# XinMing0411/AC-VAE

Measured on AMD Instinct MI355X. Metric: train-step captions/s (and audio-sec/s) at B=32, 1/2/4/8 MI355X, higher is better.
Workload: dtype f32

## Files before the change

### acvae_amd/csrc/conv.h

```cpp
#pragma once
#include <hip/hip_runtime.h>
#include <stdint.h>
#include "common.h"
#include "job_table.h"
#include "bn_bwd.h"

struct DropoutSpec {
  float p;
  const uint8_t* mask;
  uint64_t seed;
  uint32_t site;
};

enum { UP_PLAIN = 0, UP_POOL = 1, UP_DROP = 2 };

namespace acvae {
int conv3x3_igemm(const float* X, const float* scale, const float* shift, const float* Wp, float* Y, float* partials,
                  int N, int H, int W, int Cin, int Cout, hipStream_t st);
int conv_partials_rows(int N, int H, int W);
int conv3x3_igemm_bf16(const bf16_t* X, const float* scale, const float* shift, const bf16_t* Wp, bf16_t* Y,
                       float* partials, int N, int H, int W, int Cin, int Cout, hipStream_t st);
long conv3x3_wgrad_bf16_slab_floats(int N, int H, int W, int Cin, int Cout);
int conv3x3_wgrad_bf16_splits(int N, int H, int W, int Cin, int Cout);
int conv3x3_wgrad_bf16_launch(const bf16_t* dY, const bf16_t* X, const float* scale, const float* shift, float* slab, int N,
                              int H, int W, int Cin, int Cout, hipStream_t st);
int wgrad_reduce(const float* slab, int nsplit, float* dW_oihw, int Cout, int Cin, hipStream_t st);
long conv3x3_wgrad_slab_floats(int N, int H, int W, int Cin, int Cout);
int conv3x3_wgrad(const float* dY, const float* X, const float* scale, const float* shift, float* dW_oihw, float* slab,
                  int N, int H, int W, int Cin, int Cout, hipStream_t st);
bool conv3x3_wino_ok(int H, int W, int Cin, int Cout);
long conv3x3_wino_weight_floats(int Cin, int Cout);
int conv_wino_partials_rows(int N, int H, int W);
int conv3x3_wino_weights(const float* W_oihw, float* U, int Cout, int Cin, bool dgrad, hipStream_t st);
struct WinoWeightsJob { const float* W; float* U; int Cout, Cin, dgrad; };
using WinoWeightsBatch = RangeTable<WinoWeightsJob, 32>;
int conv3x3_wino_weights_batch(WinoWeightsBatch& b, hipStream_t st);
struct WinoBnReduce { const float* Y; const float* scale; const float* shift; const float* mean; const float* invstd; };
int conv3x3_wino(const float* X, const float* scale, const float* shift, const float* U, float* Y, float* partials, int N,
                 int H, int W, int Cin, int Cout, hipStream_t st, const WinoBnReduce* red = nullptr);
bool conv3x3_wino_wgrad_ok(int H, int W, int Cin, int Cout);
long conv3x3_wino_wgrad_slab_floats(int N, int H, int W, int Cin, int Cout);
int conv3x3_wino_wgrad(const float* dY, const float* X, const float* scale, const float* shift, float* dW_oihw, float* slab,
                       int N, int H, int W, int Cin, int Cout, hipStream_t st);
template <class T>
int repack_weights(const float* W_oihw, T* Wf, T* Wd, int Cout, int Cin, hipStream_t st);
struct RepackJob { const float* W; void* dst; int Cout, Cin, dgrad; };
using RepackBatch = RangeTable<RepackJob, 32>;
template <class T>
int repack_weights_batch(RepackBatch& b, hipStream_t st);
inline int conv3x3_igemm(const bf16_t* X, const float* scale, const float* shift, const bf16_t* Wp, bf16_t* Y,
                         float* partials, int N, int H, int W, int Cin, int Cout, hipStream_t st) {
  return conv3x3_igemm_bf16(X, scale, shift, Wp, Y, partials, N, H, W, Cin, Cout, st);
}
inline int conv3x3_wgrad(const bf16_t* dY, const bf16_t* X, const float* scale, const float* shift, float* dW_oihw,
                         float* slab, int N, int H, int W, int Cin, int Cout, hipStream_t st) {
  int r = conv3x3_wgrad_bf16_launch(dY, X, scale, shift, slab, N, H, W, Cin, Cout, st);
  if (r != 0) return r;
  return wgrad_reduce(slab, conv3x3_wgrad_bf16_splits(N, H, W, Cin, Cout), dW_oihw, Cout, Cin, st);
}
template <class T>
inline long conv3x3_wgrad_slab_floats_t(int N, int H, int W, int Cin, int Cout) {
  return sizeof(T) == 2 ? conv3x3_wgrad_bf16_slab_floats(N, H, W, Cin, Cout) : conv3x3_wgrad_slab_floats(N, H, W, Cin, Cout);
}
int bn0_stats(const float* x, float* partials, long rows, int F, int* nparts, hipStream_t st);
int bn0_partials_rows(long rows);
int bn_finalize(const float* partials, int P, int C, double count, const float* gamma, const float* beta,
                float* running_mean, float* running_var, int64_t* nbt, int training, float* scale, float* shift,
                float* mean, float* invstd, double* dpart, hipStream_t st);
long colsum_scratch_doubles(int width);
int colsum_tickets_reset(double* dpart, hipStream_t st);
long colsum_ticket_words();
int colsum2(const float* x, int P, int width, double* dpart, float* out, float* out2, int split, hipStream_t st);
struct ColsumJob { const float* x; int P, width; float* out; float* out_b; int R; long d0; };
using ColsumBatch = RangeTable<ColsumJob, 6, int>;
int colsum_batch(ColsumBatch& b, double* dpart, long dpart_doubles, hipStream_t st);
bool colsum_batch_plan(ColsumBatch& b, long dpart_doubles, long* dsum_doubles);
int conv1_first_blocks(int N, int T);
template <class TY>
int conv1_first_fwd(const float* x, const float* scale0, const float* shift0, const float* W1, TY* Y,
                    float* partials, int N, int T, int F, hipStream_t st);
template <class TY>
int conv1_first_bwd(const float* x, const float* scale0, const float* shift0, const float* mean0, const float* invstd0,
                    const float* W1, const TY* dY, float* dw_part, float* bn_part, float* dW1, float* dgamma0,
                    float* dbeta0, double* dpart, int N, int T, int F, hipStream_t st, const BnBwdApply* bn = nullptr);
template <class T>
int bn_relu_pool(const T* Y, const float* scale, const float* shift, T* P, int N, int H, int W, int C,
                 DropoutSpec drop, hipStream_t st, bool pool = true);
int bn_bwd_blocks(int N, int H, int W, int C);
template <class T>
int bn_bwd(const T* Y, const T* dO, int upstream, const float* scale, const float* shift, const float* mean,
           const float* invstd, float* partials, float* sum_g, float* sum_gy, T* dY, double* dpart, int N, int H,
           int W, int C, DropoutSpec drop, hipStream_t st, bool batch_stats = true, int ready_rows = 0);
template <class T>
int bn_bwd_sums(const T* Y, const T* dO, int upstream, const float* scale, const float* shift, const float* mean,
                const float* invstd, float* partials, float* sum_g, float* sum_gy, double* dpart, int N, int H, int W, int C,
                DropoutSpec drop, hipStream_t st, int ready_rows = 0);
template <class T>
int relu_mask(const T* Y, const float* scale, const float* shift, uint8_t* out, int N, int H, int W, int C, hipStream_t st);
template <class T>
int freq_mean(const T* P, float* out, long rows, int Fp, int C, hipStream_t st);
template <class T>
int freq_mean_bwd(const float* dae, T* dP, long rows, int Fp, int C, hipStream_t st);
int time_pool(const float* ae, float* out, int N, int S, int C, DropoutSpec drop, hipStream_t st);
int relu_dropout(float* x, int total, DropoutSpec drop, hipStream_t st);
}

int acvae_gemm_nt_dual(const float* A1, int64_t lda1, const float* B1, int64_t ldb1, int K1, const float* A2,
                       int64_t lda2, const float* B2, int64_t ldb2, int K2, const float* bias, float* C, int64_t ldc,
                       int M, int N, int accumulate, hipStream_t st, float* skws = nullptr);
int acvae_gemm_nt_pair(const float* A0, int64_t lda0, const float* B0, int64_t ldb0, int K0, const float* bias0, float* C0,
                       int64_t ldc0, int N0, int acc0, const float* A1, int64_t lda1, const float* B1, int64_t ldb1, int K1,
                       const float* bias1, float* C1, int64_t ldc1, int N1, int acc1, int M, hipStream_t st);
constexpr int TN_TICKETS = 256;
int acvae_gemm_tn_fused(const float* A, int64_t lda, const float* B, int64_t ldb, float* C, int64_t ldc, int M, int N, int K,
                        int accumulate, float* ws, int64_t ws_bytes, hipStream_t st);
struct TnJob {
  const float* A; long lda; const float* B; long ldb; float* C; long ldc;
  int M, N, K, k_per, slices, gx, gy, tk0;
  long slab0;
};
using TnGroup = acvae::RangeTable<TnJob, 8, int>;
bool acvae_gemm_tn_group_add(TnGroup& g, const float* A, long lda, const float* B, long ldb, float* C, long ldc, int M, int N,
                             int K);
long acvae_gemm_tn_group_plan(TnGroup& g);
int acvae_gemm_tn_group(TnGroup& g, float* ws, int64_t ws_bytes, hipStream_t st);
long acvae_skinny_ws_floats();
// ... 6 lines not shown
```

### acvae_amd/csrc/conv.hip

```cpp
#include "mfma_tile.h"
#include "../../include/acvae_hip.h"
#include "conv.h"
#include "prof.h"

namespace {
using namespace mfma;

struct FastDiv {
  unsigned long long mul;
  static FastDiv make(int d) { return FastDiv{((1ULL << 40) + (unsigned long long)d - 1) / (unsigned long long)d}; }
  __device__ __forceinline__ int div(int x) const { return (int)(((unsigned long long)(unsigned)x * mul) >> 40); }
};

struct ConvKMajorLoader {
  const float* X;
  const float* scale;
  const float* shift;
  int H, W, C, M, NC;
  FastDiv dW, dH;
  int dy, dx, ci;
  bool colok;
  float4 sc, sh;
  template <int WT>
  __device__ __forceinline__ void init(int col0) {
// ... 474 lines not shown
template <class T>
__global__ void repack_dgrad_kernel(const float* __restrict__ W, T* __restrict__ Wd, int Cout, int Cin) {
  const long total = (long)Cout * Cin * 9;
  for (long i = blockIdx.x * (long)blockDim.x + threadIdx.x; i < total; i += (long)gridDim.x * blockDim.x) {
    const int ci = (int)(i / (9 * Cout)), rem = (int)(i % (9 * Cout));
    const int tp = rem / Cout, co = rem % Cout;
    Wd[i] = (T)W[((long)co * Cin + ci) * 9 + (8 - tp)];
  }
}

template <class T>
__global__ void repack_batch_kernel(acvae::RepackBatch b) {
  const long total = b.start[b.n];
  for (long i = blockIdx.x * (long)blockDim.x + threadIdx.x; i < total; i += (long)gridDim.x * blockDim.x) {
    const int l = b.find(i);
    const acvae::RepackJob& job = b.job[l];
    const long k = i - b.start[l];
    const int Cout = job.Cout, Cin = job.Cin;
    const float* W = job.W;
    T* out = reinterpret_cast<T*>(job.dst);
    if (!job.dgrad) {
      const int co = (int)(k / (9 * Cin)), rem = (int)(k % (9 * Cin));
      const int tap = rem / Cin, ci = rem % Cin;
      out[k] = (T)W[((long)co * Cin + ci) * 9 + tap];
    } else {
      const int ci = (int)(k / (9 * Cout)), rem = (int)(k % (9 * Cout));
      const int tp = rem / Cout, co = rem % Cout;
      out[k] = (T)W[((long)co * Cin + ci) * 9 + (8 - tp)];
    }
  }
}

__global__ __launch_bounds__(256) void bn0_stats_kernel(const float* __restrict__ x, float* __restrict__ partials,
                                                        long rows, int F, int rows_per_block) {
  __shared__ float red[2][4][64];
  const int w = threadIdx.x & 63, g = threadIdx.x >> 6;
  const long r0 = (long)blockIdx.x * rows_per_block;
  float s = 0.f, q = 0.f;
  if (w < F)
    for (long r = r0 + g; r < r0 + rows_per_block && r < rows; r += 4) {
      const float v = x[r * F + w];
      s += v; q += v * v;
    }
  red[0][g][w] = s; red[1][g][w] = q;
  __syncthreads();
  if (threadIdx.x < 64 && w < F) {
    float* out = partials + (long)blockIdx.x * 2 * F;
    out[w] = red[0][0][w] + red[0][1][w] + red[0][2][w] + red[0][3][w];
    out[F + w] = red[1][0][w] + red[1][1][w] + red[1][2][w] + red[1][3][w];
  }
}

constexpr int CS_R = 64;
constexpr int CS_TICKETS = 128;
inline int cs_groups(int P) { return P < 1 ? 1 : P < 16 ? P : P <= 1024 ? 16 : P <= 4096 ? 32 : CS_R; }

struct BnFinalizeArgs {
  double count;
  const float *gamma, *beta;
  float *running_mean, *running_var;
  int64_t* nbt;
  float *scale, *shift, *mean_out, *invstd_out;
};

__device__ __forceinline__ void cs_store(double* p, double v) {
  __hip_atomic_store(reinterpret_cast<unsigned long long*>(p), (unsigned long long)__double_as_longlong(v), __ATOMIC_RELAXED,
                     __HIP_MEMORY_SCOPE_AGENT);
}
__device__ __forceinline__ double cs_load(const double* p) {
  return __longlong_as_double((long long)__hip_atomic_load(reinterpret_cast<const unsigned long long*>(p), __ATOMIC_RELAXED,
                                                           __HIP_MEMORY_SCOPE_AGENT));
}
__device__ __forceinline__ bool cs_last_arriver(unsigned* ticket, unsigned expect, int* s_last) {
  asm volatile("s_waitcnt vmcnt(0)" ::: "memory");
  __syncthreads();
  if (threadIdx.x == 0) {
    const unsigned prev = __hip_atomic_fetch_add(ticket, 1u, __ATOMIC_RELAXED, __HIP_MEMORY_SCOPE_AGENT);
    const int last = prev == expect - 1u;
    if (last) __hip_atomic_store(ticket, 0u, __ATOMIC_RELAXED, __HIP_MEMORY_SCOPE_AGENT);
    *s_last = last;
  }
  __syncthreads();
  return *s_last != 0;
}

template <bool FINALIZE>
__global__ __launch_bounds__(256) void colsum_kernel(const float* __restrict__ partials, int P, int width, double* __restrict__ dpart,
                                                     float* __restrict__ out, float* __restrict__ out2, int split,
                                                     BnFinalizeArgs bn) {
  __shared__ double red[4][64];
  __shared__ int s_last;
  unsigned* tickets = reinterpret_cast<unsigned*>(dpart);
  double* dsum = dpart + CS_TICKETS / 2;
  const int il = threadIdx.x & 63, g = threadIdx.x >> 6;
  const int i = blockIdx.x * 64 + il;
  const int R = gridDim.y;
  double a = 0.0;
  if (i < width)
    for (int p = blockIdx.y + g * R; p < P; p += 4 * R) a += (double)partials[(long)p * width + i];
  red[g][il] = a;
  __syncthreads();
  if (g == 0 && i < width) cs_store(dsum + (long)blockIdx.y * width + i, red[0][il] + red[1][il] + red[2][il] + red[3][il]);
  if (!FINALIZE) {
    if (!cs_last_arriver(tickets + blockIdx.x, (unsigned)R, &s_last)) return;
    if (g != 0 || i >= width) return;
    double t = 0.0;
    for (int r0 = 0; r0 < R; r0 += 8) {
      double v[8];
#pragma unroll
      for (int u = 0; u < 8; ++u) v[u] = r0 + u < R ? cs_load(dsum + (long)(r0 + u) * width + i) : 0.0;
#pragma unroll
      for (int u = 0; u < 8; ++u)
        if (r0 + u < R) t += v[u];
    }
    if (split > 0 && i >= split) out2[i - split] = (float)t;
    else out[i] = (float)t;
  } else {
    const int C = width >> 1, cb = C >> 6;
    const int xc = blockIdx.x % cb;
    if (!cs_last_arriver(tickets + xc, (unsigned)(2 * R), &s_last)) return;
    if (g != 0) return;
    const int c = xc * 64 + il;
    double sm = 0.0, q = 0.0;
    for (int r0 = 0; r0 < R; r0 += 8) {
      double v[8], w[8];
#pragma unroll
      for (int u = 0; u < 8; ++u) {
        v[u] = r0 + u < R ? cs_load(dsum + (long)(r0 + u) * width + c) : 0.0;
        w[u] = r0 + u < R ? cs_load(dsum + (long)(r0 + u) * width + C + c) : 0.0;
      }
#pragma unroll
      for (int u = 0; u < 8; ++u)
        if (r0 + u < R) { sm += v[u]; q += w[u]; }
    }
    const double mean = sm / bn.count;
    double var = q / bn.count - mean * mean;
    if (var < 0.0) var = 0.0;
    const float invstd = (float)(1.0 / sqrt(var + 1e-5));
    const float sc = bn.gamma[c] * invstd;
    bn.scale[c] = sc; bn.shift[c] = bn.beta[c] - (float)mean * sc;
    bn.mean_out[c] = (float)mean; bn.invstd_out[c] = invstd;
    const double unbiased = bn.count > 1.0 ? var * bn.count / (bn.count - 1.0) : var;
    bn.running_mean[c] = 0.9f * bn.running_mean[c] + 0.1f * (float)mean;
    bn.running_var[c] = 0.9f * bn.running_var[c] + 0.1f * (float)unbiased;
    if (c == 0 && bn.nbt) bn.nbt[0] += 1;
  }
}

__global__ __launch_bounds__(256) void colsum_batch_kernel(acvae::ColsumBatch b, double* __restrict__ dpart) {
  __shared__ double red[4][64];
  __shared__ int s_last;
  const int j = b.find((int)blockIdx.x);
  const acvae::ColsumJob& job = b.job[j];
  const int R = job.R;
  if ((int)blockIdx.y >= R) return;
  const float* __restrict__ partials = job.x;
  const int P = job.P, width = job.width;
  unsigned* tickets = reinterpret_cast<unsigned*>(dpart);
  double* dsum = dpart + CS_TICKETS / 2 + job.d0;
  const int il = threadIdx.x & 63, g = threadIdx.x >> 6;
  const int i = ((int)blockIdx.x - b.start[j]) * 64 + il;
  double a = 0.0;
  if (i < width)
    for (int p = blockIdx.y + g * R; p < P; p += 4 * R) a += (double)partials[(long)p * width + i];
  red[g][il] = a;
  __syncthreads();
  if (g == 0 && i < width) cs_store(dsum + (long)blockIdx.y * width + i, red[0][il] + red[1][il] + red[2][il] + red[3][il]);
  if (!cs_last_arriver(tickets + blockIdx.x, (unsigned)R, &s_last)) return;
  if (g != 0 || i >= width) return;
  double t = 0.0;
  for (int r0 = 0; r0 < R; r0 += 8) {
    double v[8];
#pragma unroll
    for (int u = 0; u < 8; ++u) v[u] = r0 + u < R ? cs_load(dsum + (long)(r0 + u) * width + i) : 0.0;
#pragma unroll
    for (int u = 0; u < 8; ++u)
      if (r0 + u < R) t += v[u];
  }
  job.out[i] = (float)t;
  if (job.out_b) job.out_b[i] = (float)t;
}

__global__ __launch_bounds__(64) void bn_eval_kernel(int C, const float* __restrict__ gamma, const float* __restrict__ beta,
                                                     const float* __restrict__ running_mean, const float* __restrict__ running_var,
                                                     float* __restrict__ scale, float* __restrict__ shift,
                                                     float* __restrict__ mean_out, float* __restrict__ invstd_out) {
  const int c = blockIdx.x * 64 + threadIdx.x;
  if (c >= C) return;
  const float invstd = 1.0f / sqrtf(running_var[c] + 1e-5f);
  const float sc = gamma[c] * invstd;
  scale[c] = sc; shift[c] = beta[c] - running_mean[c] * sc;
  mean_out[c] = running_mean[c]; invstd_out[c] = invstd;
}

constexpr int C1_RB = 8;
template <class TY>
__global__ __launch_bounds__(256) void conv1_first_fwd_kernel(const float* __restrict__ x,
                                                              const float* __restrict__ scale0,
                                                              const float* __restrict__ shift0,
                                                              const float* __restrict__ W1, TY* __restrict__ Y,
                                                              float* __restrict__ partials, int T, int F) {
  __shared__ float wl[64 * 9];
  __shared__ float patch[(C1_RB + 2) * 66];
  __shared__ float red[2][16][64];
  const int nblk_t = (T + C1_RB - 1) / C1_RB;
  const int n = blockIdx.x / nblk_t, t0 = (blockIdx.x % nblk_t) * C1_RB;
  for (int i = threadIdx.x; i < 64 * 9; i += 256) wl[i] = W1[i];
  for (int i = threadIdx.x; i < (C1_RB + 2) * 66; i += 256) {
    const int r = i / 66, cidx = i % 66;
    const int t = t0 + r - 1, w = cidx - 1;
    float v = 0.f;
    if (t >= 0 && t < T && w >= 0 && w < F) v = x[((long)n * T + t) * F + w] * scale0[w] + shift0[w];
    patch[i] = v;
  }
  __syncthreads();
  const int cq = threadIdx.x & 15, pp = threadIdx.x >> 4;
  float wreg[4][9];
#pragma unroll
  for (int c = 0; c < 4; ++c)
#pragma unroll
    for (int k = 0; k < 9; ++k) wreg[c][k] = wl[(cq * 4 + c) * 9 + k];
  float s[4] = {0, 0, 0, 0}, q[4] = {0, 0, 0, 0};
  for (int pix = pp; pix < C1_RB * 64; pix += 16) {
    const int r = pix >> 6, w = pix & 63;
    const int t = t0 + r;
    if (t >= T || w >= F) continue;
    float in[9];
#pragma unroll
    for (int k = 0; k < 9; ++k) in[k] = patch[(r + k / 3) * 66 + w + k % 3];
    float o[4];
#pragma unroll
// ... 606 lines not shown
  }
  prof_end(ACVAE_PROF_CONV_WGRAD, st);
  hipLaunchKernelGGL(wgrad_reduce_kernel, dim3(ew_grid((long)Cout * NC)), dim3(256), 0, st, slab,
                     s * wgrad_slabs_per_slice(NC, Cout), dW_oihw, Cout, Cin);
  ACVAE_LAUNCH_CHECK();
  return ACVAE_OK;
}

int wgrad_reduce(const float* slab, int nsplit, float* dW_oihw, int Cout, int Cin, hipStream_t st) {
  hipLaunchKernelGGL(wgrad_reduce_kernel, dim3(ew_grid((long)Cout * 9 * Cin)), dim3(256), 0, st, slab, nsplit, dW_oihw, Cout,
                     Cin);
  ACVAE_LAUNCH_CHECK();
  return ACVAE_OK;
}

template <class T>
int repack_weights(const float* W_oihw, T* Wf, T* Wd, int Cout, int Cin, hipStream_t st) {
  const long total = (long)Cout * Cin * 9;
  if (Wf) hipLaunchKernelGGL(repack_fwd_kernel<T>, dim3(ew_grid(total)), dim3(256), 0, st, W_oihw, Wf, Cout, Cin);
  if (Wd) hipLaunchKernelGGL(repack_dgrad_kernel<T>, dim3(ew_grid(total)), dim3(256), 0, st, W_oihw, Wd, Cout, Cin);
  ACVAE_LAUNCH_CHECK();
  return ACVAE_OK;
}
template int repack_weights<float>(const float*, float*, float*, int, int, hipStream_t);
template int repack_weights<bf16_t>(const float*, bf16_t*, bf16_t*, int, int, hipStream_t);
template <class T>
int repack_weights_batch(RepackBatch& b, hipStream_t st) {
  if (!b.ok()) return ACVAE_EINVAL;
  if (b.n <= 0) return ACVAE_OK;
  for (int l = 0; l < b.n; ++l)
    if (!b.job[l].W || !b.job[l].dst) return ACVAE_EINVAL;
  const long total = b.seal([](const RepackJob& j) { return (long)j.Cout * j.Cin * 9; });
  hipLaunchKernelGGL(repack_batch_kernel<T>, dim3(cdiv(total, 256) > 8192 ? 8192 : cdiv(total, 256)), dim3(256), 0, st, b);
  ACVAE_LAUNCH_CHECK();
  return ACVAE_OK;
}
template int repack_weights_batch<float>(RepackBatch&, hipStream_t);
template int repack_weights_batch<bf16_t>(RepackBatch&, hipStream_t);

int bn0_stats(const float* x, float* partials, long rows, int F, int* nparts, hipStream_t st) {
  if (F > 64) return ACVAE_EUNSUPPORTED;
  const int rpb = 256;
  const int nb = cdiv(rows, rpb);
  hipLaunchKernelGGL(bn0_stats_kernel, dim3(nb), dim3(256), 0, st, x, partials, rows, F, rpb);
  *nparts = nb;
  ACVAE_LAUNCH_CHECK();
  return ACVAE_OK;
}
int bn0_partials_rows(long rows) { return cdiv(rows, 256); }

int colsum2(const float* partials, int P, int width, double* dpart, float* out, float* out2, int split,
            hipStream_t st) {
  if (cdiv(width, 64) > CS_TICKETS) return ACVAE_EUNSUPPORTED;
  const int R = cs_groups(P);
  hipLaunchKernelGGL(colsum_kernel<false>, dim3(cdiv(width, 64), R), dim3(256), 0, st, partials, P, width, dpart, out, out2, split,
                     BnFinalizeArgs{});
  ACVAE_LAUNCH_CHECK();
  return ACVAE_OK;
}
bool colsum_batch_plan(ColsumBatch& b, long dpart_doubles, long* dsum_doubles) {
  long d = 0;
  for (int j = 0; j < b.n; ++j) {
    ColsumJob& c = b.job[j];
    c.R = cs_groups(c.P);
    c.d0 = d;
    d += (long)c.R * c.width;
  }
  const int blocks = b.seal([](const ColsumJob& c) { return cdiv(c.width, 64); });
  if (dsum_doubles) *dsum_doubles = d;
  return !(b.n == 1 || blocks > CS_TICKETS || CS_TICKETS / 2 + d > dpart_doubles);
}
int colsum_batch(ColsumBatch& b, double* dpart, long dpart_doubles, hipStream_t st) {
  if (!b.ok()) return ACVAE_EINVAL;
  if (b.n <= 0) return ACVAE_OK;
  if (!colsum_batch_plan(b, dpart_doubles, nullptr)) {
    for (int j = 0; j < b.n; ++j) {
      const ColsumJob& c = b.job[j];
      ACVAE_TRY(colsum2(c.x, c.P, c.width, dpart, c.out, nullptr, 0, st));
      if (c.out_b) ACVAE_TRY(colsum2(c.x, c.P, c.width, dpart, c.out_b, nullptr, 0, st));
    }
    return ACVAE_OK;
  }
  int maxr = 1;
  for (int j = 0; j < b.n; ++j)
    if (b.job[j].R > maxr) maxr = b.job[j].R;
  hipLaunchKernelGGL(colsum_batch_kernel, dim3(b.start[b.n], maxr), dim3(256), 0, st, b, dpart);
  ACVAE_LAUNCH_CHECK();
  return ACVAE_OK;
}
long colsum_scratch_doubles(int width) { return CS_TICKETS / 2 + (long)CS_R * width; }
long colsum_ticket_words() { return CS_TICKETS; }
int colsum_tickets_reset(double* dpart, hipStream_t st) {
  return hipMemsetAsync(dpart, 0, CS_TICKETS * sizeof(unsigned), st) == hipSuccess ? ACVAE_OK : (int)hipGetLastError();
}

int bn_finalize(const float* partials, int P, int C, double count, const float* gamma, const float* beta,
                float* running_mean, float* running_var, int64_t* nbt, int training, float* scale, float* shift,
                float* mean, float* invstd, double* dpart, hipStream_t st) {
  if (training) {
    if (C % 64 != 0 || cdiv(2 * C, 64) > CS_TICKETS) return ACVAE_EUNSUPPORTED;
    const int R = cs_groups(P);
    hipLaunchKernelGGL(colsum_kernel<true>, dim3(2 * C / 64, R), dim3(256), 0, st, partials, P, 2 * C, dpart, nullptr, nullptr, 0,
                       BnFinalizeArgs{count, gamma, beta, running_mean, running_var, nbt, scale, shift, mean, invstd});
  } else {
    hipLaunchKernelGGL(bn_eval_kernel, dim3(cdiv(C, 64)), dim3(64), 0, st, C, gamma, beta, running_mean, running_var, scale,
                       shift, mean, invstd);
  }
  ACVAE_LAUNCH_CHECK();
  return ACVAE_OK;
}

int conv1_first_blocks(int N, int T) { return N * cdiv(T, C1_RB); }
template <class TY>
int conv1_first_fwd(const float* x, const float* scale0, const float* shift0, const float* W1, TY* Y,
                    float* partials, int N, int T, int F, hipStream_t st) {
  if (F != 64) return ACVAE_EUNSUPPORTED;
  hipLaunchKernelGGL(conv1_first_fwd_kernel<TY>, dim3(conv1_first_blocks(N, T)), dim3(256), 0, st, x, scale0, shift0, W1,
                     Y, partials, T, F);
  ACVAE_LAUNCH_CHECK();
  return ACVAE_OK;
}
template int conv1_first_fwd<float>(const float*, const float*, const float*, const float*, float*, float*, int, int, int, hipStream_t);
template int conv1_first_fwd<bf16_t>(const float*, const float*, const float*, const float*, bf16_t*, float*, int, int, int, hipStream_t);
template <class TY>
int conv1_first_bwd(const float* x, const float* scale0, const float* shift0, const float* mean0, const float* invstd0,
                    const float* W1, const TY* dY, float* dw_part, float* bn_part, float* dW1, float* dgamma0,
                    float* dbeta0, double* dpart, int N, int T, int F, hipStream_t st, const BnBwdApply* bn) {
  if (F != 64) return ACVAE_EUNSUPPORTED;
  const int nb = conv1_first_blocks(N, T);
  if (bn) {
    if (!std::is_same<TY, float>::value) return ACVAE_EUNSUPPORTED;
    hipLaunchKernelGGL((conv1_first_bwd_kernel<float, true>), dim3(nb), dim3(256), 0, st, x, scale0, shift0, mean0, invstd0, W1,
                       (const float*)dY, dw_part, bn_part, T, F, *bn);
  } else {
    hipLaunchKernelGGL((conv1_first_bwd_kernel<TY, false>), dim3(nb), dim3(256), 0, st, x, scale0, shift0, mean0, invstd0, W1, dY,
                       dw_part, bn_part, T, F, BnBwdApply{});
  }
  ACVAE_LAUNCH_CHECK();
  ACVAE_TRY(colsum2(dw_part, nb, 576, dpart, dW1, nullptr, 0, st));
  ACVAE_TRY(colsum2(bn_part, nb, 128, dpart, dbeta0, dgamma0, 64, st));
  return ACVAE_OK;
}
template int conv1_first_bwd<float>(const float*, const float*, const float*, const float*, const float*, const float*, const float*, float*, float*, float*, float*, float*, double*, int, int, int, hipStream_t, const BnBwdApply*);
template int conv1_first_bwd<bf16_t>(const float*, const float*, const float*, const float*, const float*, const float*, const bf16_t*, float*, float*, float*, float*, float*, double*, int, int, int, hipStream_t, const BnBwdApply*);

template <class T>
int bn_relu_pool(const T* Y, const float* scale, const float* shift, T* P, int N, int H, int W, int C,
                 DropoutSpec drop, hipStream_t st, bool pool) {
  const long total = pool ? (long)N * (H / 2) * (W / 2) * (C / 4) : (long)N * H * W * (C / 4);
  if (total <= 0 || C % 4 != 0) return ACVAE_EINVAL;
  if (pool)
    hipLaunchKernelGGL(bn_relu_pool_kernel<T>, dim3(ew_grid(total)), dim3(256), 0, st, Y, scale, shift, P, N, H, W, C, drop);
  else
    hipLaunchKernelGGL(bn_relu_drop_kernel<T>, dim3(ew_grid(total)), dim3(256), 0, st, Y, scale, shift, P, N, H, W, C, drop);
  ACVAE_LAUNCH_CHECK();
// ... 124 lines not shown
```

### acvae_amd/csrc/ops_abi.hip

```cpp
#include "common.h"
#include "conv.h"
#include "rnn.h"
#include "../../include/acvae_hip.h"

namespace {
inline long al64(long x) { return (x + 63) & ~63L; }

struct ConvWs {
  long wp, partials, dpart, slab, total;
};
ConvWs conv_ws(int N, int H, int W, int Cin, int Cout) {
  ConvWs w;
  long o = 0;
  w.wp = o; o = al64(o + (long)Cout * 16 * Cin);
  long part = Cin == 1 ? (long)acvae::conv1_first_blocks(N, H) * 128 : (long)acvae::conv_partials_rows(N, H, W) * 2 * Cout;
  if (Cin > 1 && W >= 4 && W % 2 == 0 && (long)acvae::conv_wino_partials_rows(N, H, W) * 2 * Cout > part)
    part = (long)acvae::conv_wino_partials_rows(N, H, W) * 2 * Cout;
  w.partials = o; o = al64(o + part);
  w.dpart = o; o = al64(o + 2 * acvae::colsum_scratch_doubles(2 * Cout > 1024 ? 2 * Cout : 1024));
  long slab = Cin == 1 ? (long)acvae::conv1_first_blocks(N, H) * (576 + 128)
                       : acvae::conv3x3_wgrad_slab_floats(N, H, W, Cin, Cout);
  if (Cin % 64 == 0) {
    const long sb = acvae::conv3x3_wgrad_bf16_slab_floats(N, H, W, Cin, Cout);
    if (sb > slab) slab = sb;
// ... 358 lines not shown

extern "C" int acvae_lstm_step(const float* x, const float* h, const float* c, const float* w_ih, const float* w_hh,
                               const float* b_ih, const float* b_hh, float* h_out, float* c_out, void* ws_v,
                               int64_t ws_bytes, int N, int I, int H, void* stream) {
  if (N <= 0 || I <= 0 || H <= 0 || !x || !h || !c || !w_ih || !w_hh || !h_out || !c_out || !ws_v) return ACVAE_EINVAL;
  if (ws_bytes < acvae_rnn_workspace_bytes(N, 1, I, H)) return ACVAE_EWORKSPACE;
  hipStream_t st = (hipStream_t)stream;
  float* ws = (float*)ws_v;
  float* sk = ws;
  float* gates = ws + al64(acvae_skinny_ws_floats());
  ACVAE_TRY(acvae_skinny_ws_reset(sk, st));
  ACVAE_TRY(acvae_gemm_nt_dual(x, I, w_ih, I, I, nullptr, 0, nullptr, 0, 0, b_ih, gates, 4 * H, N, 4 * H, 0, st, sk));
  ACVAE_TRY(acvae_gemm_nt_dual(h, H, w_hh, H, H, nullptr, 0, nullptr, 0, 0, b_hh, gates, 4 * H, N, 4 * H, 1, st, sk));
  return acvae::lstm_fwd(gates, 4 * H, c, H, h_out, H, c_out, H, nullptr, 0, N, H, st);
}

extern "C" int acvae_bigru_seq(const float* X, const int64_t* lens, const void* const* w, float* hidden, void* ws_v,
                               int64_t ws_bytes, int N, int Tc, int E, int H, void* stream) {
  if (N <= 0 || Tc <= 0 || E <= 0 || H <= 0 || !X || !lens || !w || !hidden || !ws_v) return ACVAE_EINVAL;
  for (int i = 0; i < 8; ++i)
    if (!w[i]) return ACVAE_EINVAL;
  if (ws_bytes < acvae_rnn_workspace_bytes(N, Tc, E, H)) return ACVAE_EWORKSPACE;
  hipStream_t st = (hipStream_t)stream;
  const long R = (long)N * Tc;
  float* ws = (float*)ws_v;
  float* sk = ws;
  float* gi = ws + al64(acvae_skinny_ws_floats());
  float* gh = gi + al64(R * 8 * H);
  float* hcur = gh + al64((long)N * 4 * H);
  float* save = hcur + al64((long)N * H);
  float* hps = save + al64(R * 5 * H);
  ACVAE_TRY(acvae_skinny_ws_reset(sk, st));
  for (int dir = 0; dir < 2; ++dir) {
    const float* wih = (const float*)w[dir * 4 + 0];
    const float* whh = (const float*)w[dir * 4 + 1];
    const float* bih = (const float*)w[dir * 4 + 2];
    const float* bhh = (const float*)w[dir * 4 + 3];
    ACVAE_TRY(acvae_gemm_nt_dual(X, E, wih, E, E, nullptr, 0, nullptr, 0, 0, bih, gi, 3 * H, (int)R, 3 * H, 0, st, sk));
    ACVAE_TRY(acvae::copy_rows(hcur, H, nullptr, 0, N, H, st));
    for (int k = 0; k < Tc; ++k) {
      const int t = dir ? Tc - 1 - k : k;
      ACVAE_TRY(acvae_gemm_nt_dual(hcur, H, whh, H, H, nullptr, 0, nullptr, 0, 0, bhh, gh, 3 * H, N, 3 * H, 0, st, sk));
      ACVAE_TRY(acvae::gru_fwd(gi + (long)t * 3 * H, (long)Tc * 3 * H, gh, 3 * H, hcur, H, hcur, H,
                               hidden + (long)t * 2 * H + dir * H, (long)Tc * 2 * H, save + (long)t * 4 * H,
                               (long)Tc * 4 * H, hps + (long)t * H, (long)Tc * H, lens, t, N, H, st));
    }
  }
  return ACVAE_OK;
}

extern "C" int64_t acvae_colsum_workspace_bytes(int cols) {
  return cols > 0 ? al64(2 * acvae::colsum_scratch_doubles(cols)) * 4 : -1;
}
extern "C" int acvae_colsum(const float* x, int rows, int cols, float* out, void* ws, int64_t ws_bytes, void* stream) {
  if (!x || !out || !ws || rows <= 0 || cols <= 0) return ACVAE_EINVAL;
  if (ws_bytes < acvae_colsum_workspace_bytes(cols)) return ACVAE_EWORKSPACE;
  ACVAE_TRY(acvae::colsum_tickets_reset((double*)ws, (hipStream_t)stream));
  return acvae::colsum2(x, rows, cols, (double*)ws, out, nullptr, 0, (hipStream_t)stream);
}

static int colsum_table(int n, const int* P, const int* width, acvae::ColsumBatch& b) {
  if (n <= 0 || n > acvae::ColsumBatch::capacity || !P || !width) return ACVAE_EINVAL;
  for (int j = 0; j < n; ++j) {
    if (P[j] <= 0 || width[j] <= 0) return ACVAE_EINVAL;
    b.add({nullptr, P[j], width[j], nullptr, nullptr, 0, 0});
  }
  return ACVAE_OK;
}
extern "C" int64_t acvae_colsum_batch_workspace_bytes(int n, const int* P, const int* width) {
  acvae::ColsumBatch b;
  if (colsum_table(n, P, width, b) != ACVAE_OK) return -1;
  long d = 0;
  acvae::colsum_batch_plan(b, 0, &d);
  return ((int64_t)acvae::colsum_ticket_words() / 2 + d) * 8;
}
extern "C" int acvae_colsum_batch_plan(int n, const int* P, const int* width, int64_t ws_bytes) {
  acvae::ColsumBatch b;
  ACVAE_TRY(colsum_table(n, P, width, b));
  return acvae::colsum_batch_plan(b, (long)(ws_bytes / 8), nullptr) ? 1 : 0;
}
extern "C" int acvae_colsum_batch(int n, const void* const* x, const int* P, const int* width, const void* const* out,
                                  const void* const* out_b, void* ws, int64_t ws_bytes, int reset_tickets, void* stream) {
  acvae::ColsumBatch b;
  ACVAE_TRY(colsum_table(n, P, width, b));
  if (!x || !out || !ws) return ACVAE_EINVAL;
  for (int j = 0; j < n; ++j) {
    if (!x[j] || !out[j]) return ACVAE_EINVAL;
    b.job[j].x = (const float*)x[j];
    b.job[j].out = (float*)out[j];
    b.job[j].out_b = out_b ? (float*)out_b[j] : nullptr;
  }
  acvae::ColsumBatch plan = b;
  acvae::colsum_batch_plan(plan, 0, nullptr);
  for (int j = 0; j < n; ++j)
    if (ws_bytes < ((int64_t)acvae::colsum_ticket_words() / 2 + (int64_t)plan.job[j].R * width[j]) * 8) return ACVAE_EWORKSPACE;
  hipStream_t st = (hipStream_t)stream;
  if (reset_tickets) ACVAE_TRY(acvae::colsum_tickets_reset((double*)ws, st));
  return acvae::colsum_batch(b, (double*)ws, (long)(ws_bytes / 8), st);
}
```

### include/acvae_hip.h

```cpp
#ifndef ACVAE_HIP_H
#define ACVAE_HIP_H
#include <stdint.h>
#ifdef __cplusplus
extern "C" {
#endif

#define ACVAE_ABI_VERSION 3
int acvae_abi_version(void);

#define ACVAE_FLAG_NO_PERSIST 1
#define ACVAE_FLAG_DEFER_PARAM_GRADS 2
#define ACVAE_FLAG_NO_ATTN_SPLIT 4
#define ACVAE_FLAG_ROLLOUT_GRAD 16
#define ACVAE_FLAG_TEST_STALL 8

int acvae_persist_status_register(int device, void* status_words_host);

int acvae_gemm_nt(const float* A, int64_t lda, const float* B, int64_t ldb, const float* bias, float* C,
                  int64_t ldc, int M, int N, int K, int accumulate, void* stream);
int acvae_gemm_tn(const float* A, int64_t lda, const float* B, int64_t ldb, float* C, int64_t ldc, int M, int N,
                  int K, int accumulate, float* slab_ws, int64_t slab_ws_bytes, void* stream);
int64_t acvae_gemm_tn_workspace_bytes(int M, int N, int K);
int64_t acvae_colsum_workspace_bytes(int cols);
int acvae_colsum(const float* x, int rows, int cols, float* out, void* ws, int64_t ws_bytes, void* stream);

int64_t acvae_gemm_nt_splitk_workspace_bytes(void);
int acvae_gemm_nt_split_plan(int M, int N, int K1, int K2, int with_ws);
int acvae_gemm_nt_dual_ws(const float* A1, int64_t lda1, const float* B1, int64_t ldb1, int K1, const float* A2,
                          int64_t lda2, const float* B2, int64_t ldb2, int K2, const float* bias, float* C, int64_t ldc,
                          int M, int N, int accumulate, float* ws, int64_t ws_bytes, int reset_tickets, void* stream);
int acvae_gemm_nt_pair_c(const float* A0, int64_t lda0, const float* B0, int64_t ldb0, int K0, const float* bias0, float* C0,
                         int64_t ldc0, int N0, int acc0, const float* A1, int64_t lda1, const float* B1, int64_t ldb1, int K1,
                         const float* bias1, float* C1, int64_t ldc1, int N1, int acc1, int M, void* stream);
int64_t acvae_gemm_tn_fused_workspace_bytes(int M, int N, int K);
int acvae_gemm_tn_fused_plan(int M, int N, int K, int64_t ws_bytes);
int acvae_gemm_tn_fused_c(const float* A, int64_t lda, const float* B, int64_t ldb, float* C, int64_t ldc, int M, int N,
                          int K, int accumulate, float* ws, int64_t ws_bytes, int reset_tickets, void* stream);
int64_t acvae_gemm_tn_group_workspace_bytes(int n, const int* M, const int* N, const int* K);
int acvae_gemm_tn_group_c(int n, const void* const* A, const int64_t* lda, const void* const* B, const int64_t* ldb,
                          const void* const* C, const int64_t* ldc, const int* M, const int* N, const int* K, void* ws,
                          int64_t ws_bytes, int reset_tickets, void* stream);
int64_t acvae_colsum_batch_workspace_bytes(int n, const int* P, const int* width);
int acvae_colsum_batch_plan(int n, const int* P, const int* width, int64_t ws_bytes);
int acvae_colsum_batch(int n, const void* const* x, const int* P, const int* width, const void* const* out,
                       const void* const* out_b, void* ws, int64_t ws_bytes, int reset_tickets, void* stream);
int acvae_transpose(const float* in, int64_t ld_in, float* out, int64_t ld_out, int rows, int cols, void* stream);

int64_t acvae_attn_fwd_workspace_bytes(int N, int Tq, int S, int A, int E);
int acvae_attn_fwd(const float* qproj, int64_t q_sn, int64_t q_sj, const float* encproj, const float* enc,
                   const int64_t* lens, const float* v, float* ctx, int64_t c_sn, int64_t c_sj, float* weights,
                   int64_t w_sn, int64_t w_sj, int N, int Tq, int S, int A, int E, void* ws, int64_t ws_bytes, void* stream,
                   int flags);
int acvae_tanh_att(const float* x, float* y, int64_t n, void* stream);
int64_t acvae_attn_bwd_workspace_bytes(int N, int Tq, int S, int A);
int acvae_attn_bwd(const float* dctx, int64_t dc_sn, int64_t dc_sj, const float* qproj, int64_t q_sn, int64_t q_sj,
                   const float* encproj, const float* enc, const int64_t* lens, const float* v,
                   const float* weights, int64_t w_sn, int64_t w_sj, float* dqproj, int64_t dq_sn, int64_t dq_sj,
                   float* dencproj, float* denc, float* dv_part, float* ws, int64_t ws_bytes, int N, int Tq, int S,
                   int A, int E, void* stream);

int acvae_reparam_fwd(const float* ml, int64_t ld_ml, const float* eps, int64_t ld_eps, float* mean, float* logv,
                      float* z, int64_t ld_out, float* z2, int64_t ld_z2, int rows, int E, void* stream);
int acvae_reparam_bwd(const float* dz, int64_t ld_dz, const float* dmean_ext, const float* dlog_ext, int64_t ld_ext,
                      const float* logv, int64_t ld_lv, const float* eps, int64_t ld_eps, float* dml, int64_t ld_dml,
                      int rows, int E, void* stream);

int64_t acvae_kl_partials(int64_t n_elem);
int acvae_gauss_kl_fwd(const float* mu1, const float* lv1, const float* mu2, const float* lv2, float* partials,
                       float* out_scalar, int64_t rows, int E, void* stream);
int acvae_gauss_kl_bwd(const float* mu1, const float* lv1, const float* mu2, const float* lv2, const float* grad_out,
                       float* dmu1, float* dlv1, float* dmu2, float* dlv2, int64_t rows, int E, void* stream);

int acvae_row_logsoftmax_argmax(const float* logits, int64_t ld_n, int64_t ld_t, int64_t* argmax, float* max_logprob,
                                float* lse, int64_t o_sn, int64_t o_st, int N, int T, int V, void* stream);
#define ACVAE_SAMPLE_GREEDY 0
#define ACVAE_SAMPLE_GUMBEL 1
// ... 318 lines not shown
```

Measured before the change: 2131.

## Rework column-sum reduction with float4 row slots, contiguous row ranges and split finalize

Reworks the column-sum/BN-finalize kernels. Each group now owns a contiguous row range and reads it with float4 loads across 16-64 row slots, with an 8-deep batch of loads issued ahead. A grid z-dimension splits columns when a group has many rows, and the last-arriver finalize now reduces the partial sums across all four waves instead of one. The aim is more memory-level parallelism and a faster tail in this reduction, at the cost of larger shared-memory use, more complex ticket counts and a changed summation order.

```diff
diff --git a/acvae_amd/csrc/conv.h b/acvae_amd/csrc/conv.h
--- a/acvae_amd/csrc/conv.h
+++ b/acvae_amd/csrc/conv.h
@@ -67,11 +67,13 @@
 int bn_finalize(const float* partials, int P, int C, double count, const float* gamma, const float* beta,
                 float* running_mean, float* running_var, int64_t* nbt, int training, float* scale, float* shift,
                 float* mean, float* invstd, double* dpart, hipStream_t st);
+struct ColsumPlan { int groups, slots; long scratch; };
+ColsumPlan colsum_plan(int P, int width);
 long colsum_scratch_doubles(int width);
 int colsum_tickets_reset(double* dpart, hipStream_t st);
 long colsum_ticket_words();
 int colsum2(const float* x, int P, int width, double* dpart, float* out, float* out2, int split, hipStream_t st);
-struct ColsumJob { const float* x; int P, width; float* out; float* out_b; int R; long d0; };
+struct ColsumJob { const float* x; int P, width; float* out; float* out_b; int R, sh; long d0; };
 using ColsumBatch = RangeTable<ColsumJob, 6, int>;
 int colsum_batch(ColsumBatch& b, double* dpart, long dpart_doubles, hipStream_t st);
 bool colsum_batch_plan(ColsumBatch& b, long dpart_doubles, long* dsum_doubles);
diff --git a/acvae_amd/csrc/conv.hip b/acvae_amd/csrc/conv.hip
--- a/acvae_amd/csrc/conv.hip
+++ b/acvae_amd/csrc/conv.hip
@@ -550,8 +550,13 @@
 }
 
 constexpr int CS_R = 64;
+constexpr int CS_DEPTH = 8;
 constexpr int CS_TICKETS = 128;
 inline int cs_groups(int P) { return P < 1 ? 1 : P < 16 ? P : P <= 1024 ? 16 : P <= 4096 ? 32 : CS_R; }
+inline int cs_slot_shift(int P) {
+  const int rows = cdiv(P < 1 ? 1 : P, cs_groups(P));
+  return rows <= 16 * CS_DEPTH ? 0 : rows <= 32 * CS_DEPTH ? 1 : 2;
+}
 
 struct BnFinalizeArgs {
   double count;
@@ -582,55 +587,112 @@
   return *s_last != 0;
 }
 
+template <bool VEC>
+__device__ __forceinline__ void cs_slot_sums(const float* __restrict__ x, int r0, int r1, int width, int c0, int s, int slots,
+                                             double (&a)[4]) {
+  const int k1 = c0 + 1 < width ? 1 : 0, k2 = c0 + 2 < width ? 2 : 0, k3 = c0 + 3 < width ? 3 : 0;
+  for (int p = r0 + s; p < r1; p += slots * CS_DEPTH) {
+    float4 v[CS_DEPTH];
+#pragma unroll
+    for (int u = 0; u < CS_DEPTH; ++u) {
+      const int pu = p + u * slots;
+      const float* row = x + (long)(pu < r1 ? pu : p) * width + c0;
+      if (VEC) v[u] = *reinterpret_cast<const float4*>(row);
+      else v[u] = make_float4(row[0], row[k1], row[k2], row[k3]);
+    }
+    __builtin_amdgcn_sched_barrier(0);
+#pragma unroll
+    for (int u = 0; u < CS_DEPTH; ++u) {
+      const bool in = p + u * slots < r1;
+      a[0] += in ? (double)v[u].x : 0.0; a[1] += in ? (double)v[u].y : 0.0;
+      a[2] += in ? (double)v[u].z : 0.0; a[3] += in ? (double)v[u].w : 0.0;
+    }
+  }
+}
+__device__ __forceinline__ void cs_stage1(const float* __restrict__ x, int P, int width, int xb, int sub, int sh, int grp, int R,
+                                          double* __restrict__ dsum, double* red) {
+  const int slots = 16 << sh, cols = 64 >> sh;
+  const int q = threadIdx.x & ((cols >> 2) - 1), s = threadIdx.x >> (4 - sh);
+  const int cbase = xb * 64 + sub * cols;
+  const int c0 = cbase + q * 4;
+  const int per = P / R, rem = P % R;
+  const int r0 = grp * per + (grp < rem ? grp : rem), r1 = r0 + per + (grp < rem ? 1 : 0);
+  double a[4] = {0.0, 0.0, 0.0, 0.0};
+  if (c0 < width) {
+    if ((width & 3) == 0 && (reinterpret_cast<uintptr_t>(x) & 15) == 0) cs_slot_sums<true>(x, r0, r1, width, c0, s, slots, a);
+    else cs_slot_sums<false>(x, r0, r1, width, c0, s, slots, a);
+  }
+#pragma unroll
+  for (int c = 0; c < 4; ++c) red[s * cols + q * 4 + c] = a[c];
+  __syncthreads();
+  const int i = cbase + (int)threadIdx.x;
+  if ((int)threadIdx.x < cols && i < width) {
+    double t = red[threadIdx.x];
+#pragma unroll 8
+    for (int k = 1; k < slots; ++k) t += red[k * cols + threadIdx.x];
+    cs_store(dsum + (long)grp * width + i, t);
+  }
+}
+template <int N>
+__device__ __forceinline__ void cs_quarter(const double* __restrict__ dsum, int R, int width, const int (&col)[N], double (&t)[N]) {
+  const int per = (R + 3) >> 2, w = threadIdx.x >> 6;
+  const int lo = w * per, hi = lo + per < R ? lo + per : R;
+#pragma unroll
+  for (int k = 0; k < N; ++k) t[k] = 0.0;
+  for (int r0 = lo; r0 < hi; r0 += 8) {
+    double v[N][8];
+#pragma unroll
+    for (int u = 0; u < 8; ++u)
+#pragma unroll
+      for (int k = 0; k < N; ++k) v[k][u] = r0 + u < hi ? cs_load(dsum + (long)(r0 + u) * width + col[k]) : 0.0;
+#pragma unroll
+    for (int u = 0; u < 8; ++u)
+      if (r0 + u < hi) {
+#pragma unroll
+        for (int k = 0; k < N; ++k) t[k] += v[k][u];
+      }
+  }
+}
+__device__ __forceinline__ double cs_quarter(const double* __restrict__ dsum, int R, int width, int col) {
+  const int c[1] = {col};
+  double t[1];
+  cs_quarter<1>(dsum, R, width, c, t);
+  return t[0];
+}
+
 template <bool FINALIZE>
 __global__ __launch_bounds__(256) void colsum_kernel(const float* __restrict__ partials, int P, int width, double* __restrict__ dpart,
                                                      float* __restrict__ out, float* __restrict__ out2, int split,
                                                      BnFinalizeArgs bn) {
-  __shared__ double red[4][64];
+  __shared__ double red[16][64];
   __shared__ int s_last;
   unsigned* tickets = reinterpret_cast<unsigned*>(dpart);
   double* dsum = dpart + CS_TICKETS / 2;
   const int il = threadIdx.x & 63, g = threadIdx.x >> 6;
   const int i = blockIdx.x * 64 + il;
-  const int R = gridDim.y;
-  double a = 0.0;
-  if (i < width)
-    for (int p = blockIdx.y + g * R; p < P; p += 4 * R) a += (double)partials[(long)p * width + i];
-  red[g][il] = a;
-  __syncthreads();
-  if (g == 0 && i < width) cs_store(dsum + (long)blockIdx.y * width + i, red[0][il] + red[1][il] + red[2][il] + red[3][il]);
+  const int R = gridDim.y, sh = gridDim.z >> 1;
+  cs_stage1(partials, P, width, blockIdx.x, blockIdx.z, sh, blockIdx.y, R, dsum, &red[0][0]);
   if (!FINALIZE) {
-    if (!cs_last_arriver(tickets + blockIdx.x, (unsigned)R, &s_last)) return;
+    if (!cs_last_arriver(tickets + blockIdx.x, (unsigned)(R << sh), &s_last)) return;
+    red[g][il] = i < width ? cs_quarter(dsum, R, width, i) : 0.0;
+    __syncthreads();
     if (g != 0 || i >= width) return;
-    double t = 0.0;
-    for (int r0 = 0; r0 < R; r0 += 8) {
-      double v[8];
-#pragma unroll
-      for (int u = 0; u < 8; ++u) v[u] = r0 + u < R ? cs_load(dsum + (long)(r0 + u) * width + i) : 0.0;
-#pragma unroll
-      for (int u = 0; u < 8; ++u)
-        if (r0 + u < R) t += v[u];
-    }
+    const double t = red[0][il] + red[1][il] + red[2][il] + red[3][il];
     if (split > 0 && i >= split) out2[i - split] = (float)t;
     else out[i] = (float)t;
   } else {
     const int C = width >> 1, cb = C >> 6;
     const int xc = blockIdx.x % cb;
-    if (!cs_last_arriver(tickets + xc, (unsigned)(2 * R), &s_last)) return;
+    if (!cs_last_arriver(tickets + xc, (unsigned)(2 * R << sh), &s_last)) return;
+    const int c = xc * 64 + il;
+    const int cols[2] = {c, C + c};
+    double t2[2];
+    cs_quarter<2>(dsum, R, width, cols, t2);
+    red[g][il] = t2[0]; red[4 + g][il] = t2[1];
+    __syncthreads();
     if (g != 0) return;
-    const int c = xc * 64 + il;
-    double sm = 0.0, q = 0.0;
-    for (int r0 = 0; r0 < R; r0 += 8) {
-      double v[8], w[8];
-#pragma unroll
-      for (int u = 0; u < 8; ++u) {
-        v[u] = r0 + u < R ? cs_load(dsum + (long)(r0 + u) * width + c) : 0.0;
-        w[u] = r0 + u < R ? cs_load(dsum + (long)(r0 + u) * width + C + c) : 0.0;
-      }
-#pragma unroll
-      for (int u = 0; u < 8; ++u)
-        if (r0 + u < R) { sm += v[u]; q += w[u]; }
-    }
+    const double sm = red[0][il] + red[1][il] + red[2][il] + red[3][il];
+    const double q = red[4][il] + red[5][il] + red[6][il] + red[7][il];
     const double mean = sm / bn.count;
     double var = q / bn.count - mean * mean;
     if (var < 0.0) var = 0.0;
@@ -646,35 +708,24 @@
 }
 
 __global__ __launch_bounds__(256) void colsum_batch_kernel(acvae::ColsumBatch b, double* __restrict__ dpart) {
-  __shared__ double red[4][64];
+  __shared__ double red[16][64];
   __shared__ int s_last;
   const int j = b.find((int)blockIdx.x);
   const acvae::ColsumJob& job = b.job[j];
-  const int R = job.R;
-  if ((int)blockIdx.y >= R) return;
-  const float* __restrict__ partials = job.x;
-  const int P = job.P, width = job.width;
+  const int R = job.R, sh = job.sh;
+  if ((int)blockIdx.y >= R || (int)blockIdx.z >= 1 << sh) return;
+  const int width = job.width;
   unsigned* tickets = reinterpret_cast<unsigned*>(dpart);
   double* dsum = dpart + CS_TICKETS / 2 + job.d0;
   const int il = threadIdx.x & 63, g = threadIdx.x >> 6;
-  const int i = ((int)blockIdx.x - b.start[j]) * 64 + il;
-  double a = 0.0;
-  if (i < width)
-    for (int p = blockIdx.y + g * R; p < P; p += 4 * R) a += (double)partials[(long)p * width + i];
-  red[g][il] = a;
+  const int xb = (int)blockIdx.x - b.start[j];
+  const int i = xb * 64 + il;
+  cs_stage1(job.x, job.P, width, xb, blockIdx.z, sh, blockIdx.y, R, dsum, &red[0][0]);
+  if (!cs_last_arriver(tickets + blockIdx.x, (unsigned)(R << sh), &s_last)) return;
+  red[g][il] = i < width ? cs_quarter(dsum, R, width, i) : 0.0;
   __syncthreads();
-  if (g == 0 && i < width) cs_store(dsum + (long)blockIdx.y * width + i, red[0][il] + red[1][il] + red[2][il] + red[3][il]);
-  if (!cs_last_arriver(tickets + blockIdx.x, (unsigned)R, &s_last)) return;
   if (g != 0 || i >= width) return;
-  double t = 0.0;
-  for (int r0 = 0; r0 < R; r0 += 8) {
-    double v[8];
-#pragma unroll
-    for (int u = 0; u < 8; ++u) v[u] = r0 + u < R ? cs_load(dsum + (long)(r0 + u) * width + i) : 0.0;
-#pragma unroll
-    for (int u = 0; u < 8; ++u)
-      if (r0 + u < R) t += v[u];
-  }
+  const double t = red[0][il] + red[1][il] + red[2][il] + red[3][il];
   job.out[i] = (float)t;
   if (job.out_b) job.out_b[i] = (float)t;
 }
@@ -1387,9 +1438,9 @@
 int colsum2(const float* partials, int P, int width, double* dpart, float* out, float* out2, int split,
             hipStream_t st) {
   if (cdiv(width, 64) > CS_TICKETS) return ACVAE_EUNSUPPORTED;
-  const int R = cs_groups(P);
-  hipLaunchKernelGGL(colsum_kernel<false>, dim3(cdiv(width, 64), R), dim3(256), 0, st, partials, P, width, dpart, out, out2, split,
-                     BnFinalizeArgs{});
+  const ColsumPlan pl = colsum_plan(P, width);
+  hipLaunchKernelGGL(colsum_kernel<false>, dim3(cdiv(width, 64), pl.groups, pl.slots / 16), dim3(256), 0, st, partials, P, width,
+                     dpart, out, out2, split, BnFinalizeArgs{});
   ACVAE_LAUNCH_CHECK();
   return ACVAE_OK;
 }
@@ -1397,9 +1448,10 @@
   long d = 0;
   for (int j = 0; j < b.n; ++j) {
     ColsumJob& c = b.job[j];
-    c.R = cs_groups(c.P);
+    const ColsumPlan pl = colsum_plan(c.P, c.width);
+    c.R = pl.groups; c.sh = pl.slots >> 5;
     c.d0 = d;
-    d += (long)c.R * c.width;
+    d += pl.scratch;
   }
   const int blocks = b.seal([](const ColsumJob& c) { return cdiv(c.width, 64); });
   if (dsum_doubles) *dsum_doubles = d;
@@ -1416,12 +1468,18 @@
     }
     return ACVAE_OK;
   }
-  int maxr = 1;
-  for (int j = 0; j < b.n; ++j)
+  int maxr = 1, maxsh = 0;
+  for (int j = 0; j < b.n; ++j) {
     if (b.job[j].R > maxr) maxr = b.job[j].R;
-  hipLaunchKernelGGL(colsum_batch_kernel, dim3(b.start[b.n], maxr), dim3(256), 0, st, b, dpart);
-  ACVAE_LAUNCH_CHECK();
-  return ACVAE_OK;
+    if (b.job[j].sh > maxsh) maxsh = b.job[j].sh;
+  }
+  hipLaunchKernelGGL(colsum_batch_kernel, dim3(b.start[b.n], maxr, 1 << maxsh), dim3(256), 0, st, b, dpart);
+  ACVAE_LAUNCH_CHECK();
+  return ACVAE_OK;
+}
+ColsumPlan colsum_plan(int P, int width) {
+  const int R = cs_groups(P);
+  return {R, 16 << cs_slot_shift(P), (long)R * width};
 }
 long colsum_scratch_doubles(int width) { return CS_TICKETS / 2 + (long)CS_R * width; }
 long colsum_ticket_words() { return CS_TICKETS; }
@@ -1434,8 +1492,9 @@
                 float* mean, float* invstd, double* dpart, hipStream_t st) {
   if (training) {
     if (C % 64 != 0 || cdiv(2 * C, 64) > CS_TICKETS) return ACVAE_EUNSUPPORTED;
-    const int R = cs_groups(P);
-    hipLaunchKernelGGL(colsum_kernel<true>, dim3(2 * C / 64, R), dim3(256), 0, st, partials, P, 2 * C, dpart, nullptr, nullptr, 0,
+    const ColsumPlan pl = colsum_plan(P, 2 * C);
+    hipLaunchKernelGGL(colsum_kernel<true>, dim3(2 * C / 64, pl.groups, pl.slots / 16), dim3(256), 0, st, partials, P, 2 * C, dpart,
+                       nullptr, nullptr, 0,
                        BnFinalizeArgs{count, gamma, beta, running_mean, running_var, nbt, scale, shift, mean, invstd});
   } else {
     hipLaunchKernelGGL(bn_eval_kernel, dim3(cdiv(C, 64)), dim3(64), 0, st, C, gamma, beta, running_mean, running_var, scale,
diff --git a/acvae_amd/csrc/ops_abi.hip b/acvae_amd/csrc/ops_abi.hip
--- a/acvae_amd/csrc/ops_abi.hip
+++ b/acvae_amd/csrc/ops_abi.hip
@@ -434,6 +434,13 @@
 extern "C" int64_t acvae_colsum_workspace_bytes(int cols) {
   return cols > 0 ? al64(2 * acvae::colsum_scratch_doubles(cols)) * 4 : -1;
 }
+extern "C" int acvae_colsum_plan(int rows, int cols, int* groups, int* slots, int64_t* scratch_bytes) {
+  if (rows <= 0 || cols <= 0 || !groups || !slots || !scratch_bytes) return ACVAE_EINVAL;
+  const acvae::ColsumPlan pl = acvae::colsum_plan(rows, cols);
+  *groups = pl.groups; *slots = pl.slots;
+  *scratch_bytes = ((int64_t)acvae::colsum_ticket_words() / 2 + pl.scratch) * 8;
+  return ACVAE_OK;
+}
 extern "C" int acvae_colsum(const float* x, int rows, int cols, float* out, void* ws, int64_t ws_bytes, void* stream) {
   if (!x || !out || !ws || rows <= 0 || cols <= 0) return ACVAE_EINVAL;
   if (ws_bytes < acvae_colsum_workspace_bytes(cols)) return ACVAE_EWORKSPACE;
@@ -445,7 +452,7 @@
   if (n <= 0 || n > acvae::ColsumBatch::capacity || !P || !width) return ACVAE_EINVAL;
   for (int j = 0; j < n; ++j) {
     if (P[j] <= 0 || width[j] <= 0) return ACVAE_EINVAL;
-    b.add({nullptr, P[j], width[j], nullptr, nullptr, 0, 0});
+    b.add({nullptr, P[j], width[j], nullptr, nullptr, 0, 0, 0});
   }
   return ACVAE_OK;
 }
diff --git a/include/acvae_hip.h b/include/acvae_hip.h
--- a/include/acvae_hip.h
+++ b/include/acvae_hip.h
@@ -22,6 +22,7 @@
                   int K, int accumulate, float* slab_ws, int64_t slab_ws_bytes, void* stream);
 int64_t acvae_gemm_tn_workspace_bytes(int M, int N, int K);
 int64_t acvae_colsum_workspace_bytes(int cols);
+int acvae_colsum_plan(int rows, int cols, int* groups, int* slots, int64_t* scratch_bytes);
 int acvae_colsum(const float* x, int rows, int cols, float* out, void* ws, int64_t ws_bytes, void* stream);
 
 int64_t acvae_gemm_nt_splitk_workspace_bytes(void);
```

After: 2137, median of 6. About the same (+0.3%).
